# rhuangr/MARL-Maze

Measured on AMD Instinct MI355X. Metric: env-steps/sec (2-agent 10x10 maze) + PPO updates/sec, higher is better.
Workload: dtype f32; 1 GPU; PPO rollout+GAE+update over 65536 parallel 10x10 2-agent mazes per GPU (configs[2], the north-star workload: 65,536 parallel 10x10 mazes per GPU); mazes_per_gpu=65536, maze=10x10 (layout 19x19), horizon=16, global_batch=1048575, minibatch=209715, minibatch_steps_per_iter=25, parallelism=dp1, rollout=stream launches, gemm=x2, parity_mode=True

## Files before the change

### include/marlmaze.h

```cpp
#ifndef MARLMAZE_H
#define MARLMAZE_H

#include <stdint.h>

#ifdef __cplusplus
extern "C" {
#endif

#define MM_OBS_DIM 65
#define MM_MASK_DIM 6
#define MM_RNG_WORDS 625
#define MM_MAX_SIDE 41
#define MM_MAZES_PER_BLOCK 32

#define MM_E_ARG (-1)
#define MM_E_SIZE (-2)

#define MM_ST_GEN_FAIL 1u
#define MM_ST_BAD_MOVE 2u

typedef struct {
    int8_t x, y, dir, flags;
    int8_t lmx, lmy, olsx, olsy;
    int8_t minx, maxx, miny, maxy;
// ... 126 lines not shown
                 const float* bias, int relu, const uint32_t* mbits_in, uint32_t* mbits_out, float* colsum,
                 float cscale, float oscale, void* c, int ldc, void* stream);
int mm_x3_heads_bwd_h16(const float* dz, int J, const float* W, const uint32_t* bits, int M, int N, void* dy,
                        float* colsum, float oscale, void* stream);
int mm_gemm_a16_ok(int M, int N, int K, int lda, int ldc);
int mm_gemm_wgrad_h(int prec, int flags, const float* dy, int lddy, float dscale, const void* x, int ldx, int M, int N,
                    int K, float cscale, float* ws, float* dw, void* stream);
int mm_gemm_wgrad_partials_h(int prec, int flags, const float* dy, int lddy, float dscale, const void* x, int ldx,
                             int M, int N, int K, float cscale, float* ws, void* stream);
int mm_heads_fwd_h16(const void* h, int ldh, int K, const float* w, const float* b, int M, float* logits,
                     void* stream);
#define MM_GEMM_A_X2P 8
#define MM_GEMM_C_X2P 16
#define MM_GEMM_B_X2P 32
int mm_gemm_x2p_ok(int M, int N, int K);
int mm_x3_heads_bwd_x2p(const float* dz, int J, const float* W, const uint32_t* bits, int M, int N, void* dy,
                        float* colsum, float oscale, void* stream);
int mm_actor_front_fwd_h16(const float* ws, const float* x, int ldx, int B, int parity, void* h, void* stream);
int mm_actor_front_fwd_h16_ex(const float* ws, const float* x, int ldx, int B, int parity, void* h, int algo,
                              void* stream);

int mm_trunk3_ok(int prec, int M, int K0, int N0, int N1, int N2, int lda);
int mm_trunk3(int prec, const float* h0, int lda, int M, int K0, const uint16_t* w0, const float* b0, int N0,
              const uint16_t* w1, const float* b1, int N1, const uint16_t* w2, const float* b2, int N2, float* out,
              int ldc, void* stream);
int mm_trunk3_head_sample_ok(int prec, int M, int K0, int N0, int N1, int N2, int lda);
int mm_trunk3_head_sample(int prec, const float* h0, int lda, int M, int K0, const uint16_t* w0, const float* b0,
                          int N0, const uint16_t* w1, const float* b1, int N1, const uint16_t* w2, const float* b2,
                          int N2, const float* head_w, const float* head_b, const uint8_t* masks, uint64_t seed,
                          uint64_t offset, const uint64_t* offset_dev, int8_t* actions, float* logp,
// ... 159 lines not shown
```

### marl-maze_amd/csrc/x3mlp.hip

```cpp
#include <hip/hip_runtime.h>
#include <stdint.h>
#include <stdlib.h>

#include <algorithm>
#include <type_traits>

#include "marlmaze.h"
#include "policy_device.h"

namespace mm {
namespace x3 {

typedef __attribute__((ext_vector_type(8))) short bf16x8;
typedef __attribute__((ext_vector_type(4))) float f32x4;
typedef __attribute__((ext_vector_type(8))) _Float16 f16x8;

enum { P_X3 = MM_PREC_X3, P_F16 = MM_PREC_F16, P_X2 = MM_PREC_X2 };
template <int P>
struct Prec {
    static constexpr int kPlanes = P == P_X3 ? 3 : P == P_X2 ? 2 : 1;
    static constexpr int kBlk = 512 * kPlanes;
    static constexpr bool kScaled = P != P_X3;
};
constexpr float kX2Lo = 2048.f;
// ... 2009 lines not shown
            }
        }
    };
#pragma unroll
    for (int r = 0; r < RN; r++)
#pragma unroll
        for (int tk = 0; tk < NTK; tk++) put(acc[r * NTK + tk], accx[r * NTK + tk], RN * wave + r, tk);
#pragma unroll
    for (int e = 0; e < EX; e++) {
        const int j = wave + kWgWaves * e;
        if (j < kRem) put(acc[RN * NTK + e], accx[RN * NTK + e], kWgWaves * RN + j / NTK, j % NTK);
    }
    range_note<P>(rm);
}

__global__ __launch_bounds__(256) void k_wg_reduce(const float* __restrict__ ws, int S, long n,
                                                   float* __restrict__ out) {
    __shared__ float red[16][17];
    const int el = threadIdx.x & 15, g = threadIdx.x >> 4;
    const long e = blockIdx.x * 16L + el;
    const int per = (S + 15) / 16, s0 = g * per, s1 = min(S, s0 + per);
    float a = 0.f;
    if (e < n) {
        float v[16];
#pragma unroll
        for (int i = 0; i < 16; i++) v[i] = s0 + i < s1 ? ws[(long)(s0 + i) * n + e] : 0.f;
#pragma unroll
        for (int i = 0; i < 16; i++) a += v[i];
        for (int t = s0 + 16; t < s1; t++) a += ws[(long)t * n + e];
    }
// ... 930 lines not shown
    return (int)hipGetLastError();
}

template <int P, int C, int VW>
static int dispatch_bres_c(const float* a, int lda, float ascale, const uint16_t* b, int M, int N, int K,
                           const BresPlan& pl, const Epi& ep, hipStream_t s) {
    if (ep.c16) {
        if constexpr (P == P_F16 || (P == P_X2 && VW != 2)) {
            if (ep.mbits_out) return launch_bres<P, C, EM_FWD16, VW>(a, lda, ascale, b, M, N, K, pl, ep, s);
            if (ep.mbits_in) return launch_bres<P, C, EM_BWD16, VW>(a, lda, ascale, b, M, N, K, pl, ep, s);
        }
        return MM_E_ARG;
    }
    if (ep.mbits_out) return launch_bres<P, C, EM_FWD, VW>(a, lda, ascale, b, M, N, K, pl, ep, s);
    if (ep.mbits_in) return launch_bres<P, C, EM_BWD, VW>(a, lda, ascale, b, M, N, K, pl, ep, s);
    if constexpr (VW == 32)
        return MM_E_ARG;
    else
        return launch_bres<P, C, EM_F32, VW>(a, lda, ascale, b, M, N, K, pl, ep, s);
}

template <int P, int VW>
static int dispatch_bres(const float* a, int lda, float ascale, const uint16_t* b, int M, int N, int K,
                         const BresPlan& pl, int cfg, const Epi& ep, hipStream_t s) {
    if constexpr (P == P_X2) {
        (void)cfg;
        return dispatch_bres_c<P, C_PAIR, VW>(a, lda, ascale, b, M, N, K, pl, ep, s);
    } else {
        if constexpr (P == P_F16)
            if (cfg == C_WIDE) return dispatch_bres_c<P, C_WIDE, VW>(a, lda, ascale, b, M, N, K, pl, ep, s);
        return dispatch_bres_c<P, C_NARROW, VW>(a, lda, ascale, b, M, N, K, pl, ep, s);
    }
}

// ... 18 lines not shown
}

static int gemm_nt_f32a(int prec, const float* a, int lda, float ascale, const uint16_t* b_tp, int M, int N, int K,
                        const float* bias, int relu, const float* mask, int ldm, const uint32_t* mbits_in,
                        uint32_t* mbits_out, float* colsum, float cscale, float* c, int ldc, uint16_t* c_tp,
                        void* stream, int flags = 0, float oscale = 1.f) {
    int e = check_common(b_tp, M, N, K, mask, ldm, c, ldc, c_tp);
    if (e) return e;
    if (prec != MM_PREC_X3 && prec != MM_PREC_F16 && prec != MM_PREC_X2) return MM_E_ARG;
    const bool ap = flags & MM_GEMM_A_X2P, cp = flags & MM_GEMM_C_X2P;
    const bool a16 = flags & MM_GEMM_A_F16, c16 = flags & MM_GEMM_C_F16;
    if (flags & ~(MM_GEMM_A_F16 | MM_GEMM_C_F16 | MM_GEMM_A_X2P | MM_GEMM_C_X2P)) return MM_E_ARG;
    if (ap || cp) {
        if (prec != MM_PREC_X2 || mask || c_tp || a16 || c16) return MM_E_ARG;
        if (!a || (K & 3) || (lda & 3) || lda < K || ((uintptr_t)a & 15)) return MM_E_ARG;
        if (ap && (ascale != 1.f || (!mbits_in && !mbits_out))) return MM_E_ARG;
        if (cp && ((!mbits_out && !mbits_in) || (N & 3) || (ldc & 3) || ((uintptr_t)c & 15))) return MM_E_ARG;
        if ((mbits_in || mbits_out) && (N > 16 * 17 || (mbits_in && mbits_out))) return MM_E_ARG;
        if (mbits_in && (bias || relu)) return MM_E_ARG;
        if (colsum && (!mbits_in || !c)) return MM_E_ARG;
        if (M == 0) return 0;
        const size_t wmaxp = std::max(std::max((size_t)lda, (size_t)ldc), (size_t)N);
        const size_t capp = ((((size_t)1 << 31) - 1) / (4 * wmaxp) - 32) / kRowPad * kRowPad;
        if ((size_t)M > capp) {
            if (capp < (size_t)kRowPad) return MM_E_ARG;
            for (size_t m0 = 0; m0 < (size_t)M; m0 += capp) {
                const int mr = (int)std::min(capp, (size_t)M - m0);
                const size_t rt0 = m0 / 16;
                const int rc = gemm_nt_f32a(prec, a + m0 * lda, lda, ascale, b_tp, mr, N, K, bias, relu, nullptr, 0,
                                            mbits_in ? mbits_in + rt0 * 64 * kMaskWords : nullptr,
                                            mbits_out ? mbits_out + rt0 * 64 * kMaskWords : nullptr,
                                            colsum ? colsum + rt0 * N : nullptr, cscale, c + m0 * ldc, ldc, nullptr,
                                            stream, flags, oscale);
                if (rc) return rc;
            }
            return 0;
        }
        Epi epp{bias, nullptr, mbits_in, mbits_out, c, nullptr, colsum, ldc, 0, relu, rup(N, 32) / 32, cscale, 1,
                cp ? 1 : 0, oscale};
        hipStream_t sp = (hipStream_t)stream;
        BresPlan plp;
        int cfgp = C_PAIR;
        const bool bres = bres_enabled() && bres_plan(prec, M, N, K, lda, ldc, mbits_in || mbits_out, plp, cfgp);
        if (ap)
            return bres ? dispatch_bres<P_X2, 32>(a, lda, 1.f, b_tp, M, N, K, plp, cfgp, epp, sp)
                        : dispatch_nt<P_X2, ASrcX2PV>(a, lda, 1.f, b_tp, M, N, K, epp, sp);
        return bres ? dispatch_bres<P_X2, 4>(a, lda, ascale, b_tp, M, N, K, plp, cfgp, epp, sp)
                    : dispatch_nt<P_X2, ASrcF32>(a, lda, ascale, b_tp, M, N, K, epp, sp);
    }
    if ((a16 || c16) && (prec != MM_PREC_F16 || mask || c_tp)) return MM_E_ARG;
    if (a16 && (ascale != 1.f || (K & 3) || (lda & 3) || ((uintptr_t)a & 7))) return MM_E_ARG;
    if (c16 && ((!mbits_out && !mbits_in) || ((uintptr_t)c & 1))) return MM_E_ARG;
    if (prec == MM_PREC_X3 && (ascale != 1.f || cscale != 1.f)) return MM_E_ARG;
    const bool v4 = !a16 && !(K & 3) && !(lda & 3) && !((uintptr_t)a & 15);
    const bool v2 = !a16 && !(K & 1) && !(lda & 1) && !((uintptr_t)a & 7);
    if (!a || lda < K || !(v4 || v2 || a16) || (!v4 && !a16 && N > 64)) return MM_E_ARG;
    if ((mbits_in || mbits_out) && (N > 16 * 17 || c_tp || mask || (mbits_in && mbits_out))) return MM_E_ARG;
    if (mbits_in && (bias || relu)) return MM_E_ARG;
// ... 344 lines not shown
    hipLaunchKernelGGL((k_wgrad_dma<P_X2, TN, NTK>), dim3(rup(p.nslices, 8) * p.ncb), dim3(kWgThreads), 0, s, dy,
                       lddy, dscale, x, ldx, M, N, K, p.rows, p.nslices, p.ncb, cscale, ws);
    return (int)hipGetLastError();
}

template <int TN, int NTK>
static int launch_tr_t(const WgPlan& p, const uint32_t* dy, int lddy, const uint32_t* x, int ldx, int M, int N, int K,
                       float cscale, float* ws, hipStream_t s) {
    hipLaunchKernelGGL((k_wgrad_tr<TN, NTK>), dim3(rup(p.nslices, 8) * p.ncb), dim3(kWgThreads), 0, s, dy, lddy, x,
                       ldx, M, N, K, p.rows, p.nslices, p.ncb, cscale, ws);
    return (int)hipGetLastError();
}

static bool wg_x2p_shape(const WgPlan& p) { return p.TN == 17 && p.NTK == 9; }

template <int P, int XB = 4, int AB = 4>
static int launch_rect_p(const WgPlan& p, const float* dy, int lddy, float dscale, const float* x, int ldx, int M,
                         int N, int K, float cscale, float* ws, hipStream_t s) {
    if constexpr (P == P_X2 && XB == 4 && AB == 4) {
        const bool al = (lddy % 4 == 0) && (ldx % 4 == 0) && ((reinterpret_cast<uintptr_t>(dy) & 15) == 0) &&
                        ((reinterpret_cast<uintptr_t>(x) & 15) == 0);
        if (wg_dma_enabled() && al) {
            if (p.TN == 17 && p.NTK == 9) return launch_dma_t<17, 9>(p, dy, lddy, dscale, x, ldx, M, N, K, cscale, ws, s);
            if (p.TN == 17 && p.NTK == 8) return launch_dma_t<17, 8>(p, dy, lddy, dscale, x, ldx, M, N, K, cscale, ws, s);
        }
    }
#define MM_WR(a, b)                                                                                              \
    if (p.TN == a && p.NTK == b)                                                                                 \
        return launch_rect_t<P, a, b, XB, AB>(p, dy, lddy, dscale, x, ldx, M, N, K, cscale, ws, s);
    if constexpr (XB == 2 && P == P_X3) {
// ... 21 lines not shown
    return 1;
#endif
    if ((size_t)M * lddy * 4 >= ((size_t)1 << 31) || (size_t)M * ldx * 4 >= ((size_t)1 << 31))
        return 1;
    return prec == MM_PREC_X3   ? launch_rect_p<P_X3>(p, dy, lddy, 1.f, x, ldx, M, N, K, 1.f, ws, s)
           : prec == MM_PREC_X2 ? launch_rect_p<P_X2>(p, dy, lddy, dscale, x, ldx, M, N, K, cscale, ws, s)
                                : launch_rect_p<P_F16>(p, dy, lddy, dscale, x, ldx, M, N, K, cscale, ws, s);
}

static int gemm_wgrad(int prec, const float* dy, int lddy, float dscale, const float* x, int ldx, int M, int N, int K,
                      float cscale, float* ws, float* dw, void* stream, int flags = 0) {
    if (M < 0 || N <= 0 || K <= 0 || N > 16 * kWgMaxT || lddy < N || ldx < K) return MM_E_ARG;
    if (flags & ~(MM_GEMM_B_F16 | MM_GEMM_A_F16 | MM_GEMM_A_X2P | MM_GEMM_B_X2P)) return MM_E_ARG;
    const bool x16 = flags & MM_GEMM_B_F16, a16 = flags & MM_GEMM_A_F16;
    if (flags & (MM_GEMM_A_X2P | MM_GEMM_B_X2P)) {
        if (flags != (MM_GEMM_A_X2P | MM_GEMM_B_X2P) || prec != MM_PREC_X2 || dscale != 1.f) return MM_E_ARG;
        hipStream_t sp = (hipStream_t)stream;
        if (M == 0) return dw ? (int)hipMemsetAsync(dw, 0, sizeof(float) * (size_t)N * K, sp) : MM_E_ARG;
        if (!dy || !x || !ws || (N & 3) || (K & 3) || (lddy & 3) || (ldx & 3) ||
            (((uintptr_t)dy | (uintptr_t)x) & 15) || (size_t)M * lddy * 4 >= ((size_t)1 << 31) ||
            (size_t)M * ldx * 4 >= ((size_t)1 << 31))
            return MM_E_ARG;
        const WgPlan pp = wg_plan(prec, M, N, K);
        if (!wg_x2p_shape(pp)) return MM_E_ARG;
        const uint32_t* dyp = reinterpret_cast<const uint32_t*>(dy);
        const uint32_t* xp = reinterpret_cast<const uint32_t*>(x);
        const int ep = launch_tr_t<17, 9>(pp, dyp, lddy, xp, ldx, M, N, K, cscale, ws, sp);
        if (ep || !dw) return ep;
        const long np = (long)N * K;
        hipLaunchKernelGGL(k_wg_reduce, dim3((unsigned)((np + 15) / 16)), dim3(256), 0, sp, ws, pp.nslices, np, dw);
        return (int)hipGetLastError();
    }
    if (prec != MM_PREC_X3 && prec != MM_PREC_F16 && prec != MM_PREC_X2) return MM_E_ARG;
    if (prec == MM_PREC_X3 && (dscale != 1.f || cscale != 1.f)) return MM_E_ARG;
    hipStream_t s = (hipStream_t)stream;
    if (M == 0) return dw ? (int)hipMemsetAsync(dw, 0, sizeof(float) * (size_t)N * K, s) : MM_E_ARG;
    if (!dy || !x || !ws) return MM_E_ARG;
    const WgPlan p = wg_plan(prec, M, N, K);
    if (!p.TPW) return MM_E_ARG;
    int e = launch_wgrad_rect(prec, p, dy, lddy, dscale, x, ldx, M, N, K, cscale, ws, s, x16, a16);
    if (e == 1 && !x16 && !a16)
        e = prec == MM_PREC_X3   ? launch_wgrad<P_X3>(p, dy, lddy, 1.f, x, ldx, M, N, K, 1.f, ws, s)
// ... 26 lines not shown
                      flags);
}

extern "C" int mm_gemm_a16_ok(int M, int N, int K, int lda, int ldc) {
    BresPlan pl;
    int cfg = C_NARROW;
    return bres_enabled() && bres_plan(MM_PREC_F16, M, N, K, lda, ldc, true, pl, cfg) ? 1 : 0;
}

extern "C" int mm_gemm_x2p_ok(int M, int N, int K) {
    if (M <= 0 || N <= 0 || K <= 0 || N > 16 * kWgMaxT || (N & 3) || (K & 3)) return 0;
    if ((size_t)(M + 16) * std::max(N, K) * 4 >= ((size_t)1 << 31)) return 0;
    return wg_x2p_shape(wg_plan(MM_PREC_X2, M, N, K)) ? 1 : 0;
}

extern "C" int mm_gemm_wgrad_slices(int prec, int M, int N, int K) {
    if (M <= 0 || N <= 0 || K <= 0 || (prec != MM_PREC_X3 && prec != MM_PREC_F16 && prec != MM_PREC_X2))
        return MM_E_ARG;
    const WgPlan p = wg_plan(prec, M, N, K);
    return p.TPW ? p.nslices : MM_E_ARG;
}

extern "C" int mm_gemm_wgrad_partials(int prec, const float* dy, int lddy, float dscale, const float* x, int ldx, int M,
                                      int N, int K, float cscale, float* ws, void* stream) {
    if (M <= 0) return MM_E_ARG;
    return gemm_wgrad(prec, dy, lddy, dscale, x, ldx, M, N, K, cscale, ws, nullptr, stream);
}

extern "C" int mm_critic_update_ok(int M, int K0, int ldx) {
    if (M <= 0 || K0 <= 128 || K0 > 132 || (K0 & 1) || (ldx & 1) || ldx < K0) return 0;
// ... 38 lines not shown
```

### marl-maze_amd/marlmaze/_lib.py

```python
import ctypes
import os

import torch

PKG_ROOT = os.path.dirname(os.path.dirname(os.path.abspath(__file__)))
LIB_PATH = os.environ.get("MARLMAZE_LIB") or os.path.join(PKG_ROOT, "libmarlmaze.so")

OBS_DIM = 65
MASK_DIM = 6
RNG_WORDS = 625
MAX_SIDE = 41
MAZES_PER_BLOCK = 32

ST_GEN_FAIL = 1
ST_BAD_MOVE = 2

GAE_AUTO, GAE_COLUMN, GAE_WALK, GAE_SCAN = 0, 1, 2, 3

ACT_SAMPLE, ACT_GREEDY = 0, 1
ACT_MODES = {"sample": ACT_SAMPLE, "greedy": ACT_GREEDY}

EVAL_WORDS = 32
EV_EPISODES, EV_SOLVED, EV_TIMEOUTS, EV_SUM_LEN, EV_SUM_LEN_SOLVED, EV_SUM_SHORT_SOLVED = 0, 1, 2, 3, 4, 5
EV_MIN_LEN_SOLVED, EV_MAX_LEN_SOLVED, EV_SUM_RATIO_Q16, EV_BAD_SHORT = 6, 7, 8, 9
# ... 23 lines not shown
           "mm_actor_front_ws_len", "mm_actor_front_prep", "mm_actor_front_fwd", "mm_actor_front_fwd_ex",
           "mm_actor_front_grad_len", "mm_actor_front_partial_len", "mm_actor_front_bwd", "mm_actor_front_bwd_ex",
           "mm_actor_front_bwd_to", "mm_actor_front_bwd_grid",
           "mm_x3_tp_len", "mm_x3_tp_pack", "mm_x3_nt", "mm_x3_nt_f32a", "mm_x3_mbits_len",
           "mm_x3_heads_bwd", "mm_ppo_loss_partials", "mm_ppo_loss", "mm_ppo_loss_bwd",
           "mm_gemm_tp_len", "mm_gemm_tp_pack", "mm_gemm_nt", "mm_gemm_nt_algo", "mm_gemm_wgrad_algo", "mm_gemm_wgrad_ws_len",
           "mm_gemm_wgrad", "mm_colsum", "mm_mse_loss_partials", "mm_mse_loss", "mm_losses_final",
           "mm_clip_adam_ws_len", "mm_clip_adam", "mm_gemm_tp_pack_multi", "mm_gemm_wgrad_slices",
           "mm_gemm_wgrad_partials", "mm_colsum_multi_ws_len", "mm_colsum_multi", "mm_wsum_multi", "mm_critic_value",
           "mm_gemm_range_flag", "mm_gemm_nt_h", "mm_gemm_a16_ok", "mm_gemm_wgrad_h", "mm_gemm_wgrad_partials_h",
           "mm_heads_fwd_h16", "mm_x3_heads_bwd_h16", "mm_trunk3_ok", "mm_trunk3",
           "mm_trunk3_head_sample_ok", "mm_trunk3_head_sample", "mm_actor_front_fwd_h16",
           "mm_actor_front_fwd_h16_ex", "mm_head_act", "mm_act", "mm_eval_init", "mm_eval_accum",
           "mm_env_dist", "mm_env_par", "mm_par_init", "mm_par_accum",
           "mm_elog_state_words", "mm_elog_init", "mm_elog_start", "mm_elog_step",
           "mm_gemm_x2p_ok", "mm_x3_heads_bwd_x2p",
           "mm_critic_update_ok", "mm_critic_update")
VERSION = 308

PREC_X3, PREC_F16, PREC_X2 = 0, 1, 2
FRONT_BWD = {"mfma": 0, "valu": 1}
FRONT_FWD = {"row1": 0, "row2": 1, "mfma": 2}
GEMM_ALGO = {"auto": 0, "stream": 1}
GEMM_A_F16, GEMM_C_F16, GEMM_B_F16 = 1, 2, 4
GEMM_A_X2P, GEMM_C_X2P, GEMM_B_X2P = 8, 16, 32


class EnvDesc(ctypes.Structure):
    _fields_ = [
        ("n", ctypes.c_int32), ("size_w", ctypes.c_int32), ("size_h", ctypes.c_int32),
        ("max_timestep", ctypes.c_int32), ("difficulty", ctypes.c_int32),
# ... 176 lines not shown
        L.mm_gemm_range_flag.argtypes = [P, i32, P]
        L.mm_gemm_range_flag.restype = i32
        for name, args in (("mm_gemm_nt_h", [i32, i32, P, i32, f32, P, i32, i32, i32, P, i32, P, P, P, f32, f32, P, i32,
                                             P]),
                           ("mm_x3_heads_bwd_h16", [P, i32, P, P, i32, i32, P, P, f32, P]),
                           ("mm_gemm_a16_ok", [i32, i32, i32, i32, i32]),
                           ("mm_gemm_wgrad_h", [i32, i32, P, i32, f32, P, i32, i32, i32, i32, f32, P, P, P]),
                           ("mm_gemm_wgrad_partials_h", [i32, i32, P, i32, f32, P, i32, i32, i32, i32, f32, P, P]),
                           ("mm_heads_fwd_h16", [P, i32, i32, P, P, i32, P, P]),
                           ("mm_trunk3_ok", [i32, i32, i32, i32, i32, i32, i32]),
                           ("mm_trunk3", [i32, P, i32, i32, i32, P, P, i32, P, P, i32, P, P, i32, P, i32, P]),
                           ("mm_trunk3_head_sample_ok", [i32, i32, i32, i32, i32, i32, i32]),
                           ("mm_actor_front_fwd_h16", [P, P, i32, i32, i32, P, P]),
                           ("mm_actor_front_fwd_h16_ex", [P, P, i32, i32, i32, P, i32, P]),
                           ("mm_gemm_x2p_ok", [i32, i32, i32]),
                           ("mm_x3_heads_bwd_x2p", [P, i32, P, P, i32, i32, P, P, f32, P]),
                           ("mm_critic_update_ok", [i32, i32, i32]),
                           ("mm_critic_update", [P, i32, i32, i32] + [P] * 18),
                           ("mm_trunk3_head_sample", [i32, P, i32, i32, i32, P, P, i32, P, P, i32, P, P, i32, P, P, P,
                                                      u64, u64, P, P, P, P, P, P, i32, P])):
            if hasattr(L, name):
                getattr(L, name).argtypes = args
                getattr(L, name).restype = i32
        L.mm_colsum_multi_ws_len.argtypes = [ctypes.POINTER(ColsumSeg), i32]
        L.mm_colsum_multi_ws_len.restype = ctypes.c_long
        L.mm_colsum_multi.argtypes = [ctypes.POINTER(ColsumSeg), i32, P, P]
        L.mm_colsum_multi.restype = i32
        L.mm_wsum_multi.argtypes = [ctypes.POINTER(WsumSeg), i32, P]
        L.mm_wsum_multi.restype = i32
        L.mm_x3_mbits_len.argtypes = [i32]
# ... 74 lines not shown
```

### marl-maze_amd/marlmaze/networks.py

```python
import ctypes
import math
import os

import numpy as np
import torch
import torch.nn as nn
import torch.nn.functional as F

FEATURE_DIMS = [4, 4, 4, 4, 4, 4, 4, 4, 4, 4, 4, 4, 2, 2, 1, 4, 1, 1, 1, 1, 1, 1, 2]
FEATURE_AMOUNT = len(FEATURE_DIMS)
OBS_SPACE = int(np.sum(FEATURE_DIMS))
EMBEDDING_DIM = 20
KQ_DIM = 10
_SQRT_KQ = float(np.sqrt(KQ_DIM))


class Projection(nn.Module):

    def __init__(self, parity_mode=True):
        super().__init__()
        self.layers = nn.ModuleList([nn.Linear(d, EMBEDDING_DIM) for d in FEATURE_DIMS])
        self.parity_mode = parity_mode
        starts = np.zeros(FEATURE_AMOUNT, np.int64) if parity_mode else np.cumsum([0] + FEATURE_DIMS[:-1])
        self.register_buffer("_starts", torch.as_tensor(starts), persistent=False)
# ... 128 lines not shown
    from . import x3

    s = _grad_scale(dy.shape[0], prec)
    if x3.is_planes(dy):
        return x3.wgrad(dy, x, prec=prec, dscale=1.0, cscale=1.0 / s, out=out, nk=nk)
    if dy.dtype == torch.float16:
        return x3.wgrad(dy.contiguous(), x, prec=prec, dscale=1.0, cscale=1.0 / s, out=out)
    return x3.wgrad(dy.contiguous(), x, prec=prec, dscale=s, out=out)


F16_ACT = os.environ.get("MARLMAZE_F16_ACT", "1") != "0"
F16_H0 = os.environ.get("MARLMAZE_F16_H0", "1") != "0"


X2_PLANES = os.environ.get("MARLMAZE_X2_PLANES", "1") != "0"

CRITIC_FUSED = os.environ.get("MARLMAZE_CRITIC_FUSED", "1") != "0"


class _SavedPlanes(torch.Tensor):

    _STORAGE = ("as_subclass",)

    @staticmethod
    def __new__(cls, p):
        return torch.Tensor._make_subclass(cls, p)

    def planes(self):
        return self.as_subclass(torch.Tensor)

# ... 65 lines not shown
    s = _grad_scale(M, prec)
    grads = [None] * (2 * L)
    dx = None
    for l in range(L - 1, -1, -1):
        g16 = dy.dtype == torch.float16
        o_w, o_b = (outs[2 * l], outs[2 * l + 1]) if outs is not None else (None, None)
        grads[2 * l] = _wgrad(dy, hs[l], prec, out=o_w, nk=tuple(ws[l].shape))
        assert cs is not None or not g16, "an fp16 dY comes with its column sums"
        grads[2 * l + 1] = x3.colsum(dy if cs is None else cs, out=o_b)
        wt = x3.pack(ws[l], trans=True, prec=prec)
        ascale, cscale = (1.0, 1.0 / s) if g16 else (s, None)
        if l > 0:
            cs = x3.colsum_buf(M, ws[l].shape[1], dy.device)
            out = torch.empty((M, ws[l].shape[1]), dtype=torch.float16, device=dy.device) if g16 else None
            if x3.is_planes(dy):
                out = x3.planes(M, ws[l].shape[1], dy.device) if x3.is_planes(hs[l - 1]) else None
            dy = x3.gemm(dy, wt, mbits_in=ctx_bits[l - 1], colsum=cs, ascale=ascale, cscale=cscale, out=out,
                         oscale=s)
        elif need_dx:
            dx = x3.gemm(dy, wt, ascale=ascale, cscale=cscale)
    return dx, grads


def _g16(prec, hs, ws, need_dx):
    from . import x3

    M = hs[0].shape[0]
    if prec != "f16" or hs[-1].dtype != torch.float16:
        return False
    shapes = [(w.shape[1], w.shape[0]) for w in ws[1:]] + ([(ws[0].shape[1], ws[0].shape[0])] if need_dx else [])
    return all(n % 4 == 0 and k % 4 == 0 and x3.a16_ok(M, n, k) for n, k in shapes)
# ... 481 lines not shown
```

### marl-maze_amd/marlmaze/x3.py

```python
import weakref

import torch

from . import _lib


PRECS = {"x3": _lib.PREC_X3, "f16": _lib.PREC_F16, "x2": _lib.PREC_X2}


class TP:
    __slots__ = ("buf", "R", "C", "prec", "src")

    def __init__(self, R, C, device, buf=None, prec="x3"):
        self.R, self.C, self.prec = int(R), int(C), prec
        self.src = None
        n = _lib.lib().mm_gemm_tp_len(PRECS[prec], self.R, self.C)
        self.buf = buf if buf is not None else torch.empty(n, dtype=torch.int16, device=device)
        assert self.buf.numel() >= n

    def ptr(self):
        return _lib.ptr(self.buf)


_PACK_CACHE = {}
# ... 241 lines not shown
    return t is not None and t.dim() == 4 and t.dtype == torch.float16 and t.shape[2:] == (2, 4)


def _plane_rows(t):
    return t.stride()[1:] == (8, 4, 1) and t.stride(0) % 8 == 0


def _pitch(t):
    return t.stride(0) // 2 if is_planes(t) else t.stride(0)


def x2p_ok(M, N, K):
    return bool(_lib.lib().mm_gemm_x2p_ok(int(M), int(N), int(K)))


def a16_ok(M, N, K):
    return bool(_lib.lib().mm_gemm_a16_ok(int(M), int(N), int(K), int(K), int(N)))


def range_flag(out=None, clear=True):
    if out is None:
        out = torch.empty(1, dtype=torch.int32, device="cuda")
    _lib.check(_lib.lib().mm_gemm_range_flag(_lib.ptr(out), int(bool(clear)), _lib.stream_ptr()),
               "mm_gemm_range_flag")
    return out


def set_algo(name):
    prev = _lib.lib().mm_gemm_nt_algo(_lib.GEMM_ALGO[name])
    return {v: k for k, v in _lib.GEMM_ALGO.items()}[prev]


WGRAD_ALGO = {"dma": 0, "reg": 1}


def set_wgrad_algo(name):
    prev = _lib.lib().mm_gemm_wgrad_algo(WGRAD_ALGO[name])
    return {v: k for k, v in WGRAD_ALGO.items()}[prev]


def wgrad(dy, x, prec="x3", dscale=1.0, out=None, checked=False, cscale=None, nk=None):
    if is_planes(dy) or is_planes(x):
        assert is_planes(dy) and is_planes(x) and prec == "x2" and not checked and float(dscale) == 1.0
        N, K = nk
        M = dy.shape[0]
        assert x.shape[0] == M and _plane_rows(dy) and _plane_rows(x)
        assert dy.shape[1] == N // 4 and x.shape[1] == K // 4, (dy.shape, x.shape, nk)
        flags = _lib.GEMM_A_X2P | _lib.GEMM_B_X2P
    elif checked and prec != "x3":
        if dy.dtype == torch.float16 or x.dtype == torch.float16 or cscale is not None:
            raise ValueError("wgrad(checked=True) takes fp32 dY and X without cscale (the x3 redo's forms)")
        range_flag(clear=True)
        res = wgrad(dy, x, prec, dscale, out)
        if int(range_flag(clear=True).item()):
            res = wgrad(dy, x, "x3", 1.0, out)
        return res
    else:
        M, N = dy.shape
        K = x.shape[1]
        assert x.shape[0] == M and dy.stride(1) == 1 and x.stride(1) == 1
        assert x.dtype in (torch.float32, torch.float16) and dy.dtype in (torch.float32, torch.float16), \
            (x.dtype, dy.dtype)
        flags = ((_lib.GEMM_B_F16 if x.dtype == torch.float16 else 0)
# ... 113 lines not shown
```

Baseline: 7.545 million env-steps/s.

## Keep first-layer backward dY in x2 planes with mixed-input wgrad kernel

Adds a new wgrad kernel that takes dY in pre-split x2 plane format and the fp32 layer input X, converting X to x2 planes in LDS with an optional double-buffered overlap of conversion and MFMA. The layer-1 backward GEMM can now emit planes output even when the layer-0 input is plain fp32, so the first-layer weight gradient avoids splitting dY from fp32 again. It also enables the plain-planes-A path in the GEMM dispatcher (EM_F32 with VW=32). The change adds kernel complexity and an extra plane-format intermediate whose shape eligibility is gated by new check functions.

Measured after the change: 7.672 million env-steps/s, median of 6. 1.7% higher.

```diff
diff --git a/include/marlmaze.h b/include/marlmaze.h
--- a/include/marlmaze.h
+++ b/include/marlmaze.h
@@ -164,6 +164,7 @@
 #define MM_GEMM_C_X2P 16
 #define MM_GEMM_B_X2P 32
 int mm_gemm_x2p_ok(int M, int N, int K);
+int mm_gemm_x2p_dy_ok(int M, int N, int K);
 int mm_x3_heads_bwd_x2p(const float* dz, int J, const float* W, const uint32_t* bits, int M, int N, void* dy,
                         float* colsum, float oscale, void* stream);
 int mm_actor_front_fwd_h16(const float* ws, const float* x, int ldx, int B, int parity, void* h, void* stream);
diff --git a/marl-maze_amd/csrc/x3mlp.hip b/marl-maze_amd/csrc/x3mlp.hip
--- a/marl-maze_amd/csrc/x3mlp.hip
+++ b/marl-maze_amd/csrc/x3mlp.hip
@@ -2047,6 +2047,296 @@
     range_note<P>(rm);
 }
 
+#ifndef WG_MIX_OVERLAP
+#define WG_MIX_OVERLAP 1
+#endif
+template <int TN, int NTK>
+__global__ __launch_bounds__(kWgThreads) void k_wgrad_mix(const uint32_t* __restrict__ dy, int lddy,
+                                                          const float* __restrict__ x, int ldx, int M, int N, int K,
+                                                          int rows, int nslices, int ncb, float cscale,
+                                                          float* __restrict__ ws) {
+    constexpr int P = P_X2;
+    constexpr int kB = Prec<P>::kBlk;
+    constexpr int RN = TN / kWgWaves;
+    constexpr int kRem = (TN - kWgWaves * RN) * NTK;
+    constexpr int EX = (kRem + kWgWaves - 1) / kWgWaves;
+    static_assert(RN > 0 && (kRem == 0 || TN - kWgWaves * RN == 1), "leftover tiles of one n-tile (one A fragment)");
+    constexpr int wpA = tr_pitch(TN);
+    constexpr int kWB = 16 * NTK;
+    constexpr int kSecA = 32 * wpA, kSecB = 32 * kWB / 4;
+    static_assert(kSecA % 64 == 0 && kSecB % 64 == 0, "parts of whole DMA instructions");
+    constexpr int kInsA = kSecA / 64, kInsB = kSecB / 64;
+    constexpr int kImg = NTK * kB;
+    constexpr bool kOverlap = WG_MIX_OVERLAP != 0;
+    constexpr int kImgs = kOverlap ? 2 : 1;
+    constexpr int itemsB = 64 * NTK;
+    constexpr int kPerB = (itemsB + kWgThreads - 1) / kWgThreads;
+    static_assert(2 * (kSecA + kSecB) * 16 + kImgs * kImg * 2 <= 160 * 1024, "LDS");
+    __shared__ __attribute__((aligned(16))) uint4 rawA[2 * kSecA];
+    __shared__ __attribute__((aligned(16))) uint4 rawB[2 * kSecB];
+    __shared__ __attribute__((aligned(16))) uint16_t img[kImgs * kImg];
+    const int lane = threadIdx.x & 63;
+    const int wave = __builtin_amdgcn_readfirstlane(threadIdx.x >> 6);
+    const int xcd = blockIdx.x & 7, slot = blockIdx.x >> 3;
+    const int s = (slot / ncb) * 8 + xcd, cb = slot % ncb;
+    if (s >= nslices) return;
+    const int m_begin = s * rows, nrows = min(M, m_begin + rows) - m_begin;
+    const int col0 = cb * NTK * 16;
+#ifdef WG_MIX_NO_SKIP
+    constexpr int live = NTK;
+#else
+    const int live = min(NTK, (K - col0 + 15) / 16);
+#endif
+    __amdgpu_buffer_rsrc_t rsA = __builtin_amdgcn_make_buffer_rsrc(
+        (void*)(dy + (size_t)m_begin * lddy), (short)0, (int)(nrows * lddy * 4), 0x00020000);
+    __amdgpu_buffer_rsrc_t rsB = __builtin_amdgcn_make_buffer_rsrc(
+        (void*)(x + (size_t)m_begin * ldx + col0), (short)0, (int)((nrows * ldx - col0) * 4), 0x00020000);
+    asm volatile("" : "+s"(rsA));
+    asm volatile("" : "+s"(rsB));
+
+    constexpr int kSlotA = (kInsA + kWgWaves - 1) / kWgWaves, kSlotB = (kInsB + kWgWaves - 1) / kWgWaves;
+    uint32_t obA[2][kSlotA], obB[2][kSlotB];
+#pragma unroll
+    for (int k = 0; k < kSlotA; k++) {
+        const int e = 64 * min(wave + kWgWaves * k, kInsA - 1) + lane;
+        const int r = e / wpA, c = e % wpA;
+#pragma unroll
+        for (int t = 0; t < 2; t++) {
+            obA[t][k] = c < 4 * TN ? (uint32_t)(((32 * t + r) * lddy + 4 * c) * 4) : kBufOOB;
+            asm volatile("" : "+v"(obA[t][k]));
+        }
+    }
+#pragma unroll
+    for (int k = 0; k < kSlotB; k++) {
+        const int e = 64 * min(wave + kWgWaves * k, kInsB - 1) + lane;
+        const int r = e / (kWB / 4), c4 = e % (kWB / 4);
+#pragma unroll
+        for (int t = 0; t < 2; t++) {
+            obB[t][k] = (uint32_t)(((32 * t + r) * ldx + 4 * c4) * 4);
+            asm volatile("" : "+v"(obB[t][k]));
+        }
+    }
+    const uint32_t stepA = 2u * 32u * (uint32_t)lddy * 4u, stepB = 2u * 32u * (uint32_t)ldx * 4u;
+    auto issueA = [&](auto tc, int st) {
+        constexpr int T = decltype(tc)::value;
+        const uint32_t base = lds_addr(rawA + T * kSecA);
+        __builtin_amdgcn_sched_barrier(0);
+#pragma unroll
+        for (int k = 0; k < kSlotA; k++) {
+            const int a = wave + kWgWaves * k;
+            if (a < kInsA) {
+                if (st >= 2) asm volatile("v_add_u32 %0, %0, %1" : "+v"(obA[T][k]) : "s"(stepA));
+                dma16(rsA, obA[T][k], base + 1024u * (uint32_t)a);
+            }
+        }
+        __builtin_amdgcn_sched_barrier(0);
+    };
+    auto issueB = [&](auto tc, int st) {
+        constexpr int T = decltype(tc)::value;
+        const uint32_t base = lds_addr(rawB + T * kSecB);
+        __builtin_amdgcn_sched_barrier(0);
+#pragma unroll
+        for (int k = 0; k < kSlotB; k++) {
+            const int bi = wave + kWgWaves * k;
+            if (bi < kInsB) {
+                if (st >= 2) asm volatile("v_add_u32 %0, %0, %1" : "+v"(obB[T][k]) : "s"(stepB));
+                dma16(rsB, obB[T][k], base + 1024u * (uint32_t)bi);
+            }
+        }
+        __builtin_amdgcn_sched_barrier(0);
+    };
+    constexpr int kRemA = kInsA % kWgWaves, kRemB = kInsB % kWgWaves;
+    static_assert(kRemA != 0 && kRemB == 0, "waves below kRemA issue one more instruction (of dY)");
+    constexpr int kInsW = kSlotA + kSlotB, kInsWmin = kInsW - 1;
+    auto wait_stage = [&](bool later_in_flight) {
+        asm volatile("" ::: "memory");
+        __builtin_amdgcn_sched_barrier(0);
+        if (later_in_flight) {
+            if (wave < kRemA) {
+                __builtin_amdgcn_s_waitcnt(0x0F70 | (kInsW & 15) | ((kInsW >> 4) << 14));
+            } else {
+                __builtin_amdgcn_s_waitcnt(0x0F70 | (kInsWmin & 15) | ((kInsWmin >> 4) << 14));
+            }
+        } else {
+            __builtin_amdgcn_s_waitcnt(0x0F70);
+        }
+        __builtin_amdgcn_sched_barrier(0);
+        asm volatile("" ::: "memory");
+    };
+    auto barrier = [&]() {
+        __builtin_amdgcn_sched_barrier(0);
+        __builtin_amdgcn_s_waitcnt((15 << 0) | (7 << 4) | (0 << 8) | (3 << 14));
+        __builtin_amdgcn_s_barrier();
+        asm volatile("" ::: "memory");
+        __builtin_amdgcn_sched_barrier(0);
+    };
+    auto convB = [&](const float* xs, uint16_t* im) {
+#pragma unroll
+        for (int q = 0; q < kPerB; q++) {
+            const int e = threadIdx.x + kWgThreads * q;
+            if (e < itemsB) {
+                const int c = e / kWB, j = e - c * kWB;
+                const float* src = xs + 8 * c * kWB + j;
+                float v[8];
+#pragma unroll
+                for (int i = 0; i < 8; i++) v[i] = src[i * kWB];
+                const int loff = (j >> 4) * kB + c * 128 + (j & 15) * 8;
+                store_piece_x2_plain<false>(v, 1.f, reinterpret_cast<uint4*>(im + loff));
+            }
+        }
+    };
+    auto fragB = [&](const uint16_t* im, int tile, bf16x8 (&f)[3]) {
+        const bf16x8* p = reinterpret_cast<const bf16x8*>(im + tile * kB) + lane;
+#pragma unroll
+        for (int q = 0; q < 2; q++) f[q] = p[64 * q];
+    };
+    const int tc = lane >> 4, tq = (lane >> 2) & 3, tp = lane & 3;
+    const uint32_t laneA = (uint32_t)(16 * ((8 * tc + tq) * wpA + tp));
+    typedef short s4v __attribute__((ext_vector_type(4)));
+    auto tr = [&](const char* p) {
+        return __builtin_amdgcn_ds_read_tr16_b64_v4i16((__attribute__((address_space(3))) s4v*)(p));
+    };
+    auto fragA = [&](const char* stage, int tile, bf16x8 (&f)[3]) {
+        const char* p = stage + laneA + 64 * tile;
+        constexpr int r4 = 16 * 4 * wpA;
+#pragma unroll
+        for (int q = 0; q < 2; q++) {
+            const s4v u = tr(p + 8 * q), v = tr(p + 8 * q + r4);
+            f[q] = bf16x8{u[0], u[1], u[2], u[3], v[0], v[1], v[2], v[3]};
+        }
+    };
+
+    f32x4 acc[RN * NTK + EX], accx[RN * NTK + EX];
+#pragma unroll
+    for (int u = 0; u < RN * NTK + EX; u++) acc[u] = accx[u] = f32x4{0.f, 0.f, 0.f, 0.f};
+    const int nsteps = (nrows + 31) / 32;
+    constexpr std::integral_constant<int, 0> c0{};
+    constexpr std::integral_constant<int, 1> c1{};
+    auto mfmas = [&](const uint16_t* im, const bf16x8 (&a)[RN][3], const bf16x8 (&ax)[3], bf16x8 (&b)[2][3],
+                     auto&& mid) {
+#pragma unroll
+        for (int tk = 0; tk < NTK; tk++) {
+            if (tk + 1 < NTK) fragB(im, tk + 1, b[(tk + 1) & 1]);
+            if (tk < live) {
+#pragma unroll
+                for (int r = 0; r < RN; r++)
+                    acc[r * NTK + tk] = mma<P>(a[r], b[tk & 1], acc[r * NTK + tk], accx[r * NTK + tk]);
+            }
+            if (tk == 0) mid();
+        }
+#pragma unroll
+        for (int e = 0; e < EX; e++) {
+            int j = wave + kWgWaves * e;
+            j = j < kRem ? j : kRem - 1;
+            if (j % NTK < live) {
+                bf16x8 b1[3];
+                fragB(im, j % NTK, b1);
+                acc[RN * NTK + e] = mma<P>(ax, b1, acc[RN * NTK + e], accx[RN * NTK + e]);
+            }
+        }
+    };
+    if constexpr (!kOverlap) {
+        issueA(c0, 0);
+        issueB(c0, 0);
+        if (nsteps > 1) {
+            issueA(c1, 1);
+            issueB(c1, 1);
+        }
+        wait_stage(nsteps > 1);
+        barrier();
+        convB(reinterpret_cast<const float*>(rawB), img);
+        barrier();
+        auto step = [&](auto tcur, int st) {
+            constexpr int T = decltype(tcur)::value;
+            const char* stage = reinterpret_cast<const char*>(rawA + T * kSecA);
+            bf16x8 a[RN][3], ax[3], b[2][3];
+#pragma unroll
+            for (int r = 0; r < RN; r++) fragA(stage, RN * wave + r, a[r]);
+            if constexpr (EX > 0) fragA(stage, kWgWaves * RN, ax);
+            fragB(img, 0, b[0]);
+            barrier();
+            if (st + 2 < nsteps) {
+                issueA(tcur, st + 2);
+                issueB(tcur, st + 2);
+            }
+            mfmas(img, a, ax, b, [] {});
+            if (st + 1 < nsteps) {
+                wait_stage(st + 2 < nsteps);
+                barrier();
+                convB(reinterpret_cast<const float*>(rawB + (1 - T) * kSecB), img);
+                barrier();
+            }
+        };
+        for (int st = 0; st < nsteps; st += 2) {
+            step(c0, st);
+            if (st + 1 < nsteps) step(c1, st + 1);
+        }
+    } else {
+        issueA(c0, 0);
+        issueB(c0, 0);
+        if (nsteps > 1) issueB(c1, 1);
+        wait_stage(false);
+        barrier();
+        convB(reinterpret_cast<const float*>(rawB), img);
+        auto step = [&](auto tcur, int st) {
+            constexpr int T = decltype(tcur)::value;
+            constexpr std::integral_constant<int, 1 - T> cn{};
+            barrier();
+            if (st + 1 < nsteps) issueA(cn, st + 1);
+            if (st + 2 < nsteps) issueB(tcur, st + 2);
+            const char* stage = reinterpret_cast<const char*>(rawA + T * kSecA);
+            const uint16_t* im = img + T * kImg;
+            bf16x8 a[RN][3], ax[3], b[2][3];
+#pragma unroll
+            for (int r = 0; r < RN; r++) fragA(stage, RN * wave + r, a[r]);
+            if constexpr (EX > 0) fragA(stage, kWgWaves * RN, ax);
+            fragB(im, 0, b[0]);
+            mfmas(im, a, ax, b, [&] {
+                if (st + 1 < nsteps)
+                    convB(reinterpret_cast<const float*>(rawB + (1 - T) * kSecB), img + (1 - T) * kImg);
+            });
+            wait_stage(false);
+        };
+        for (int st = 0; st < nsteps; st += 2) {
+            step(c0, st);
+            if (st + 1 < nsteps) step(c1, st + 1);
+        }
+    }
+    __builtin_amdgcn_s_waitcnt(0x0F70);
+#pragma unroll
+    for (int t = 0; t < 2; t++) {
+#pragma unroll
+        for (int k = 0; k < kSlotA; k++) asm volatile("" ::"v"(obA[t][k]));
+#pragma unroll
+        for (int k = 0; k < kSlotB; k++) asm volatile("" ::"v"(obB[t][k]));
+    }
+    asm volatile("" ::"s"(rsA), "s"(rsB), "s"(stepA), "s"(stepB));
+    uint32_t rm = 0;
+    float* out = ws + (size_t)s * N * K;
+    auto put = [&](f32x4 v, f32x4 vx, int tn, int tk) {
+        v = x2_combine<P>(v, vx);
+        const int col = col0 + 16 * tk + (lane & 15);
+#pragma unroll
+        for (int g = 0; g < 4; g++) {
+            const int row = 16 * tn + 4 * (lane >> 4) + g;
+            if (row < N && col < K) {
+                rm = max(rm, __float_as_uint(v[g]) & 0x7FFFFFFFu);
+                out[(size_t)row * K + col] = v[g] * cscale;
+            }
+        }
+    };
+#pragma unroll
+    for (int r = 0; r < RN; r++)
+#pragma unroll
+        for (int tk = 0; tk < NTK; tk++) put(acc[r * NTK + tk], accx[r * NTK + tk], RN * wave + r, tk);
+#pragma unroll
+    for (int e = 0; e < EX; e++) {
+        const int j = wave + kWgWaves * e;
+        if (j < kRem) put(acc[RN * NTK + e], accx[RN * NTK + e], kWgWaves * RN + j / NTK, j % NTK);
+    }
+    range_note<P>(rm);
+}
+
 __global__ __launch_bounds__(256) void k_wg_reduce(const float* __restrict__ ws, int S, long n,
                                                    float* __restrict__ out) {
     __shared__ float red[16][17];
@@ -3007,10 +3297,7 @@
     }
     if (ep.mbits_out) return launch_bres<P, C, EM_FWD, VW>(a, lda, ascale, b, M, N, K, pl, ep, s);
     if (ep.mbits_in) return launch_bres<P, C, EM_BWD, VW>(a, lda, ascale, b, M, N, K, pl, ep, s);
-    if constexpr (VW == 32)
-        return MM_E_ARG;
-    else
-        return launch_bres<P, C, EM_F32, VW>(a, lda, ascale, b, M, N, K, pl, ep, s);
+    return launch_bres<P, C, EM_F32, VW>(a, lda, ascale, b, M, N, K, pl, ep, s);
 }
 
 template <int P, int VW>
@@ -3059,16 +3346,17 @@
     if (ap || cp) {
         if (prec != MM_PREC_X2 || mask || c_tp || a16 || c16) return MM_E_ARG;
         if (!a || (K & 3) || (lda & 3) || lda < K || ((uintptr_t)a & 15)) return MM_E_ARG;
-        if (ap && (ascale != 1.f || (!mbits_in && !mbits_out))) return MM_E_ARG;
+        const bool plain_a = ap && !mbits_in && !mbits_out;
+        if (ap && ascale != 1.f) return MM_E_ARG;
         if (cp && ((!mbits_out && !mbits_in) || (N & 3) || (ldc & 3) || ((uintptr_t)c & 15))) return MM_E_ARG;
         if ((mbits_in || mbits_out) && (N > 16 * 17 || (mbits_in && mbits_out))) return MM_E_ARG;
         if (mbits_in && (bias || relu)) return MM_E_ARG;
         if (colsum && (!mbits_in || !c)) return MM_E_ARG;
-        if (M == 0) return 0;
+        if (M == 0) return plain_a ? MM_E_ARG : 0;
         const size_t wmaxp = std::max(std::max((size_t)lda, (size_t)ldc), (size_t)N);
         const size_t capp = ((((size_t)1 << 31) - 1) / (4 * wmaxp) - 32) / kRowPad * kRowPad;
         if ((size_t)M > capp) {
-            if (capp < (size_t)kRowPad) return MM_E_ARG;
+            if (capp < (size_t)kRowPad || plain_a) return MM_E_ARG;
             for (size_t m0 = 0; m0 < (size_t)M; m0 += capp) {
                 const int mr = (int)std::min(capp, (size_t)M - m0);
                 const size_t rt0 = m0 / 16;
@@ -3087,6 +3375,7 @@
         BresPlan plp;
         int cfgp = C_PAIR;
         const bool bres = bres_enabled() && bres_plan(prec, M, N, K, lda, ldc, mbits_in || mbits_out, plp, cfgp);
+        if (plain_a && !bres) return MM_E_ARG;
         if (ap)
             return bres ? dispatch_bres<P_X2, 32>(a, lda, 1.f, b_tp, M, N, K, plp, cfgp, epp, sp)
                         : dispatch_nt<P_X2, ASrcX2PV>(a, lda, 1.f, b_tp, M, N, K, epp, sp);
@@ -3461,6 +3750,16 @@
 
 static bool wg_x2p_shape(const WgPlan& p) { return p.TN == 17 && p.NTK == 9; }
 
+template <int TN, int NTK>
+static int launch_mix_t(const WgPlan& p, const uint32_t* dy, int lddy, const float* x, int ldx, int M, int N, int K,
+                        float cscale, float* ws, hipStream_t s) {
+    hipLaunchKernelGGL((k_wgrad_mix<TN, NTK>), dim3(rup(p.nslices, 8) * p.ncb), dim3(kWgThreads), 0, s, dy, lddy, x,
+                       ldx, M, N, K, p.rows, p.nslices, p.ncb, cscale, ws);
+    return (int)hipGetLastError();
+}
+
+static bool wg_mix_shape(const WgPlan& p) { return p.TN == 17 && p.NTK == 8; }
+
 template <int P, int XB = 4, int AB = 4>
 static int launch_rect_p(const WgPlan& p, const float* dy, int lddy, float dscale, const float* x, int ldx, int M,
                          int N, int K, float cscale, float* ws, hipStream_t s) {
@@ -3512,18 +3811,21 @@
     if (flags & ~(MM_GEMM_B_F16 | MM_GEMM_A_F16 | MM_GEMM_A_X2P | MM_GEMM_B_X2P)) return MM_E_ARG;
     const bool x16 = flags & MM_GEMM_B_F16, a16 = flags & MM_GEMM_A_F16;
     if (flags & (MM_GEMM_A_X2P | MM_GEMM_B_X2P)) {
-        if (flags != (MM_GEMM_A_X2P | MM_GEMM_B_X2P) || prec != MM_PREC_X2 || dscale != 1.f) return MM_E_ARG;
+        const bool mix = flags == MM_GEMM_A_X2P;
+        if ((!mix && flags != (MM_GEMM_A_X2P | MM_GEMM_B_X2P)) || prec != MM_PREC_X2 || dscale != 1.f)
+            return MM_E_ARG;
         hipStream_t sp = (hipStream_t)stream;
         if (M == 0) return dw ? (int)hipMemsetAsync(dw, 0, sizeof(float) * (size_t)N * K, sp) : MM_E_ARG;
-        if (!dy || !x || !ws || (N & 3) || (K & 3) || (lddy & 3) || (ldx & 3) ||
+        if (!dy || !x || !ws || (N & 3) || (!mix && (K & 3)) || (lddy & 3) || (ldx & 3) ||
             (((uintptr_t)dy | (uintptr_t)x) & 15) || (size_t)M * lddy * 4 >= ((size_t)1 << 31) ||
             (size_t)M * ldx * 4 >= ((size_t)1 << 31))
             return MM_E_ARG;
         const WgPlan pp = wg_plan(prec, M, N, K);
-        if (!wg_x2p_shape(pp)) return MM_E_ARG;
+        if (!(mix ? wg_mix_shape(pp) : wg_x2p_shape(pp))) return MM_E_ARG;
         const uint32_t* dyp = reinterpret_cast<const uint32_t*>(dy);
         const uint32_t* xp = reinterpret_cast<const uint32_t*>(x);
-        const int ep = launch_tr_t<17, 9>(pp, dyp, lddy, xp, ldx, M, N, K, cscale, ws, sp);
+        const int ep = mix ? launch_mix_t<17, 8>(pp, dyp, lddy, x, ldx, M, N, K, cscale, ws, sp)
+                           : launch_tr_t<17, 9>(pp, dyp, lddy, xp, ldx, M, N, K, cscale, ws, sp);
         if (ep || !dw) return ep;
         const long np = (long)N * K;
         hipLaunchKernelGGL(k_wg_reduce, dim3((unsigned)((np + 15) / 16)), dim3(256), 0, sp, ws, pp.nslices, np, dw);
@@ -3580,6 +3882,21 @@
     return wg_x2p_shape(wg_plan(MM_PREC_X2, M, N, K)) ? 1 : 0;
 }
 
+static bool x2p_plain_a_ok(int M, int N, int K, int lda, int ldc) {
+    if (M <= 0 || N <= 0 || K <= 0 || (N & 3) || (lda & 3) || lda < N || ldc < K) return false;
+    const size_t wmax = std::max(std::max((size_t)lda, (size_t)ldc), (size_t)K);
+    if ((size_t)M > ((((size_t)1 << 31) - 1) / (4 * wmax) - 32) / kRowPad * kRowPad) return false;
+    BresPlan pl;
+    int cfg = C_PAIR;
+    return bres_enabled() && bres_plan(MM_PREC_X2, M, K, N, lda, ldc, false, pl, cfg);
+}
+
+extern "C" int mm_gemm_x2p_dy_ok(int M, int N, int K) {
+    if (M <= 0 || N <= 0 || K <= 0 || N > 16 * kWgMaxT || (N & 3) || (K & 3)) return 0;
+    if ((size_t)(M + 16) * std::max(N, K) * 4 >= ((size_t)1 << 31)) return 0;
+    return wg_mix_shape(wg_plan(MM_PREC_X2, M, N, K)) && x2p_plain_a_ok(M, N, K, N, K) ? 1 : 0;
+}
+
 extern "C" int mm_gemm_wgrad_slices(int prec, int M, int N, int K) {
     if (M <= 0 || N <= 0 || K <= 0 || (prec != MM_PREC_X3 && prec != MM_PREC_F16 && prec != MM_PREC_X2))
         return MM_E_ARG;
diff --git a/marl-maze_amd/marlmaze/_lib.py b/marl-maze_amd/marlmaze/_lib.py
--- a/marl-maze_amd/marlmaze/_lib.py
+++ b/marl-maze_amd/marlmaze/_lib.py
@@ -61,7 +61,7 @@
            "mm_actor_front_fwd_h16_ex", "mm_head_act", "mm_act", "mm_eval_init", "mm_eval_accum",
            "mm_env_dist", "mm_env_par", "mm_par_init", "mm_par_accum",
            "mm_elog_state_words", "mm_elog_init", "mm_elog_start", "mm_elog_step",
-           "mm_gemm_x2p_ok", "mm_x3_heads_bwd_x2p",
+           "mm_gemm_x2p_ok", "mm_gemm_x2p_dy_ok", "mm_x3_heads_bwd_x2p",
            "mm_critic_update_ok", "mm_critic_update")
 VERSION = 308
 
@@ -268,6 +268,7 @@
                            ("mm_actor_front_fwd_h16", [P, P, i32, i32, i32, P, P]),
                            ("mm_actor_front_fwd_h16_ex", [P, P, i32, i32, i32, P, i32, P]),
                            ("mm_gemm_x2p_ok", [i32, i32, i32]),
+                           ("mm_gemm_x2p_dy_ok", [i32, i32, i32]),
                            ("mm_x3_heads_bwd_x2p", [P, i32, P, P, i32, i32, P, P, f32, P]),
                            ("mm_critic_update_ok", [i32, i32, i32]),
                            ("mm_critic_update", [P, i32, i32, i32] + [P] * 18),
diff --git a/marl-maze_amd/marlmaze/networks.py b/marl-maze_amd/marlmaze/networks.py
--- a/marl-maze_amd/marlmaze/networks.py
+++ b/marl-maze_amd/marlmaze/networks.py
@@ -166,6 +166,7 @@
 
 
 X2_PLANES = os.environ.get("MARLMAZE_X2_PLANES", "1") != "0"
+X2_DY1 = os.environ.get("MARLMAZE_X2_DY1", "1") != "0"
 
 CRITIC_FUSED = os.environ.get("MARLMAZE_CRITIC_FUSED", "1") != "0"
 
@@ -261,7 +262,9 @@
             cs = x3.colsum_buf(M, ws[l].shape[1], dy.device)
             out = torch.empty((M, ws[l].shape[1]), dtype=torch.float16, device=dy.device) if g16 else None
             if x3.is_planes(dy):
-                out = x3.planes(M, ws[l].shape[1], dy.device) if x3.is_planes(hs[l - 1]) else None
+                below = x3.is_planes(hs[l - 1]) or (l == 1 and X2_PLANES and X2_DY1 and hs[0].dtype == torch.float32
+                                                    and x3.x2p_dy_ok(M, *ws[0].shape))
+                out = x3.planes(M, ws[l].shape[1], dy.device) if below else None
             dy = x3.gemm(dy, wt, mbits_in=ctx_bits[l - 1], colsum=cs, ascale=ascale, cscale=cscale, out=out,
                          oscale=s)
         elif need_dx:
diff --git a/marl-maze_amd/marlmaze/x3.py b/marl-maze_amd/marlmaze/x3.py
--- a/marl-maze_amd/marlmaze/x3.py
+++ b/marl-maze_amd/marlmaze/x3.py
@@ -279,6 +279,10 @@
     return bool(_lib.lib().mm_gemm_x2p_ok(int(M), int(N), int(K)))
 
 
+def x2p_dy_ok(M, N, K):
+    return bool(_lib.lib().mm_gemm_x2p_dy_ok(int(M), int(N), int(K)))
+
+
 def a16_ok(M, N, K):
     return bool(_lib.lib().mm_gemm_a16_ok(int(M), int(N), int(K), int(K), int(N)))
 
@@ -306,12 +310,16 @@
 
 def wgrad(dy, x, prec="x3", dscale=1.0, out=None, checked=False, cscale=None, nk=None):
     if is_planes(dy) or is_planes(x):
-        assert is_planes(dy) and is_planes(x) and prec == "x2" and not checked and float(dscale) == 1.0
+        assert is_planes(dy) and prec == "x2" and not checked and float(dscale) == 1.0
         N, K = nk
         M = dy.shape[0]
-        assert x.shape[0] == M and _plane_rows(dy) and _plane_rows(x)
-        assert dy.shape[1] == N // 4 and x.shape[1] == K // 4, (dy.shape, x.shape, nk)
-        flags = _lib.GEMM_A_X2P | _lib.GEMM_B_X2P
+        assert x.shape[0] == M and _plane_rows(dy) and dy.shape[1] == N // 4, (dy.shape, x.shape, nk)
+        if is_planes(x):
+            assert _plane_rows(x) and x.shape[1] == K // 4, (x.shape, nk)
+            flags = _lib.GEMM_A_X2P | _lib.GEMM_B_X2P
+        else:
+            assert x.dtype == torch.float32 and x.dim() == 2 and x.stride(1) == 1 and x.shape[1] == K, (x.shape, nk)
+            flags = _lib.GEMM_A_X2P
     elif checked and prec != "x3":
         if dy.dtype == torch.float16 or x.dtype == torch.float16 or cscale is not None:
             raise ValueError("wgrad(checked=True) takes fp32 dY and X without cscale (the x3 redo's forms)")
```
